# Nyrox/raymond

Measured on AMD Instinct MI355X. Metric: Msamples/s (whole node) + achieved HBM GB/s, 1920x1080 @ 500spp 5-bounce, higher is better.
Workload: dtype f64

## Files before the change

include/raymond_hip_probe.h:

```cpp
#ifndef RAYMOND_HIP_PROBE_H
#define RAYMOND_HIP_PROBE_H

#include "raymond_hip.h"

#ifdef __cplusplus
extern "C" {
#endif

rmd_status rmd_probe_philox4x32_10(rmd_context *ctx, size_t n, const uint32_t *ctr4, const uint32_t *key2, uint32_t *out4);
rmd_status rmd_probe_block_uniforms(rmd_context *ctx, uint64_t seed, size_t n, const uint32_t *pixel, const uint32_t *sample,
                                    const uint32_t *block, double *out5);
rmd_status rmd_probe_sphere_intersect(rmd_context *ctx, size_t n, const double *sphere4, const double *ray6, int32_t *hit, double *t);
rmd_status rmd_probe_sphere_normal(rmd_context *ctx, size_t n, const double *sphere4, const double *ray6, const double *t, double *n3);
rmd_status rmd_probe_plane_intersect(rmd_context *ctx, size_t n, const double *plane6, const double *ray6, int32_t *hit, double *t);
rmd_status rmd_probe_aabb_intersect(rmd_context *ctx, size_t n, const double *aabb6, const double *ray6, int32_t *hit, double *t);
rmd_status rmd_probe_triangle_intersect(rmd_context *ctx, size_t n, const double *pos9, const double *ray6, int32_t *hit, double *t);
rmd_status rmd_probe_triangle_normal(rmd_context *ctx, size_t n, const double *pos9, const double *nrm9, const double *ray6,
                                     const double *t, double *n3);
rmd_status rmd_probe_onb(rmd_context *ctx, size_t n, const double *n3, double *t3, double *b3);
rmd_status rmd_probe_cosine_hemisphere(rmd_context *ctx, size_t n, const double *r1, const double *r2, double *dir3, double *pdf);
rmd_status rmd_probe_importance_sample_ggx(rmd_context *ctx, size_t n, const double *reflect3, const double *rough, const double *r1,
                                           const double *r2, double *dir3);
rmd_status rmd_probe_ggx_distribution(rmd_context *ctx, size_t n, const double *n3, const double *h3, const double *rough, double *out);
rmd_status rmd_probe_geometry_smith(rmd_context *ctx, size_t n, const double *n3, const double *v3, const double *l3,
// ... 5 lines not shown
rmd_status rmd_probe_scene_intersect(rmd_context *ctx, const rmd_scene *scene, size_t n, const double *ray6, int32_t *obj, double *t,
                                     uint32_t *sub);
rmd_status rmd_probe_grid_intersect(rmd_context *ctx, const rmd_scene *scene, uint32_t g, size_t n, const double *ray6, int32_t *hit,
                                    double *t, uint32_t *tri);
rmd_status rmd_probe_grid_intersect_deep(rmd_context *ctx, const rmd_scene *scene, uint32_t g, size_t n, const double *ray6, uint32_t cut_lanes,
                                         uint32_t cut_round, uint32_t rays_per_wave, int32_t *hit, double *t, uint32_t *tri);
rmd_status rmd_probe_trace_samples(rmd_context *ctx, const rmd_scene *scene, const rmd_camera *cam, const rmd_settings *settings,
                                   size_t n, const uint32_t *xy2, const uint32_t *sample, double *rgb_out, int32_t *path_obj,
                                   uint32_t *path_sub);

rmd_status rmd_probe_triangle_sphere(size_t n, const double *pos9, double *out5);
rmd_status rmd_probe_primary_candidates(const rmd_camera *cam, const rmd_settings *settings, const rmd_object *objects, uint32_t n_objects, uint32_t n_grids,
                                        int64_t axis_pairs_tunable, size_t n_tiles, const uint32_t *tiles4, uint64_t *launch3, uint64_t *out2);
rmd_status rmd_probe_launch_plan(uint32_t mode, uint32_t grid, size_t n, const uint32_t *in5, uint64_t *out8);
rmd_status rmd_probe_launch_sizes(uint32_t mode, uint32_t grid, uint64_t *out8);
rmd_status rmd_probe_scene_layout(const rmd_scene *scene, uint32_t *n_objects, uint32_t *n_grids, uint32_t *mask_words_total);
#define RMD_PROBE_SCRATCH_FORMS 7u
#define RMD_PROBE_SCRATCH_PARTS 14u
rmd_status rmd_probe_denoise_scratch(uint32_t form, uint32_t width, uint32_t height, uint32_t n_rects, uint32_t guided, uint32_t n_cands, uint64_t n_table,
                                     uint64_t *out3, uint64_t *total);
rmd_status rmd_probe_pretest_pairs(rmd_context *ctx, size_t n, const double *sphere5, const double *pos9, const double *ray6, int32_t *pass,
                                   int32_t *hit, double *t);

#ifdef __cplusplus
}
#endif
#endif
```

raymond_amd/csrc/api.cpp:

```cpp
#define RMD_WITH_HIP 1
#include <algorithm>
#include <cmath>
#include <limits>
#include <cstdio>
#include <cstdlib>
#include <cstring>
#include <new>

#include "internal.hpp"
#include "launch.hpp"

using rmd::bind;

namespace {
thread_local std::string tl_last_error;

rmd_status context_create(int32_t device, hipStream_t stream, bool own_stream, rmd_context **out) {
	if (!out) return rmd::fail(nullptr, RMD_ERR_INVALID_ARGUMENT, "rmd_context_create: null out pointer");
	*out = nullptr;
	int count = 0;
	hipError_t e = hipGetDeviceCount(&count);
	if (e != hipSuccess || count <= 0)
		return rmd::fail(nullptr, RMD_ERR_NO_DEVICE, std::string("no HIP device: ") + (e != hipSuccess ? hipGetErrorString(e) : "device count is 0"));
	if (device < 0 || device >= count) return rmd::fail(nullptr, RMD_ERR_INVALID_ARGUMENT, "rmd_context_create: device ordinal out of range");
// ... 21 lines not shown
			return v ? (int64_t)std::atoll(v) : 0;
		};
		ctx->tunable[RMD_TUNE_SAMPLE_SPLIT] = env_int("RMD_SAMPLE_SPLIT");
		ctx->tunable[RMD_TUNE_WALK_BATCH] = env_int("RMD_WALK_BATCH");
		ctx->tunable[RMD_TUNE_MASK_BUDGET] = env_int("RMD_MASK_BUDGET");
		ctx->tunable[RMD_TUNE_SCRATCH_CAP_MB] = env_int("RMD_SCRATCH_CAP_MB");
		ctx->tunable[RMD_TUNE_WALK_CUT] = env_int("RMD_WALK_CUT");
		ctx->tunable[RMD_TUNE_SPLIT_MIN_SAMPLES] = env_int("RMD_SPLIT_MIN_SAMPLES");
		ctx->tunable[RMD_TUNE_CHAIN_ITEMS] = env_int("RMD_CHAIN_ITEMS");
		ctx->tunable[RMD_TUNE_AXIS_PAIRS] = env_int("RMD_AXIS_PAIRS");
		ctx->tunable[RMD_TUNE_PATH_QUEUES] = env_int("RMD_PATH_QUEUES");
		const char *form = std::getenv("RMD_LAUNCH_FORM");
		ctx->tunable[RMD_TUNE_LAUNCH_FORM] = !form ? 0 : (std::strcmp(form, "per-item") == 0 || std::strcmp(form, "1") == 0) ? 1 : (std::strcmp(form, "persistent") == 0 || std::strcmp(form, "2") == 0) ? 2 : 0;
#if RMD_DIAG
		ctx->debug_flags = (uint32_t)env_int("RMD_DEBUG");
#endif
	}
	if (hipEventCreate(&ctx->ev_start) != hipSuccess || hipEventCreate(&ctx->ev_stop) != hipSuccess)
		return rmd::fail(nullptr, RMD_ERR_HIP, "hipEventCreate failed");
	{
		void *h = nullptr, *d = nullptr;
		hipError_t fe = hipHostMalloc(&h, rmd::kFaultWords * sizeof(uint32_t), hipHostMallocMapped);
		if (fe == hipSuccess) {
			ctx->h_fault = (uint32_t *)h;
			std::memset(h, 0, rmd::kFaultWords * sizeof(uint32_t));
			fe = hipHostGetDevicePointer(&d, h, 0);
		}
		if (fe != hipSuccess) return rmd::fail(nullptr, RMD_ERR_HIP, std::string("fault words (hipHostMalloc): ") + hipGetErrorString(fe));
		ctx->d_fault = (uint32_t *)d;
	}
// ... 532 lines not shown
		const uint32_t waves_per_slot = has_grid ? 256u : 24u;
		k = (waves_per_slot * ctx->wave_slots + n_wave_tiles - 1u) / n_wave_tiles;
		if (has_grid && k < 2u) k = 2u;
		uint32_t min_samples = has_grid ? (sample_count <= rmd::kChainMaxSamples && ctx->tunable[RMD_TUNE_CHAIN_ITEMS] != 1 ? 2u : rmd::kSplitMinSamplesGrid) : 64u;
		if (ctx->tunable[RMD_TUNE_SPLIT_MIN_SAMPLES] > 0) min_samples = (uint32_t)std::min<int64_t>(ctx->tunable[RMD_TUNE_SPLIT_MIN_SAMPLES], 1 << 20);
		if (k > sample_count / min_samples) k = sample_count / min_samples;
		if (has_grid && k < 2u && sample_count >= 4u && ctx->tunable[RMD_TUNE_SPLIT_MIN_SAMPLES] <= 0) k = 2u;
	}
	if (k > 64u) k = 64u;
	while (k > 1u && (uint64_t)n_wave_tiles * k > 0x7FFFFFFFull) k--;
	if (k < 2u) k = 1u;
	if (buffered) *buffered = k > 1u || may_buffer_unsplit;
	return k;
}

static rmd_status render_tiles_async_impl(rmd_context *ctx, const rmd_scene *scene, const rmd_camera *camera, const rmd_settings *settings,
                                          const rmd_tile_rect *tiles, uint32_t n_tiles, double *accum_dev, double *accum_sq_dev) {
	if (rmd_status s = bind(ctx)) return s;
	if (rmd_status s = check_render_args(ctx, scene, camera, settings)) return s;
	if (!accum_dev || (n_tiles && !tiles)) return rmd::fail(ctx, RMD_ERR_INVALID_ARGUMENT, "rmd_render_tiles: null tiles/accum pointer");
	if (rmd_status s = prepare_wave_tiles(ctx, camera, tiles, n_tiles)) return s;
	if (settings->bounce_limit == 0u) {
		RMD_HIP(ctx, hipEventRecord(ctx->ev_start, ctx->stream));
		RMD_HIP(ctx, hipEventRecord(ctx->ev_stop, ctx->stream));
		ctx->timed = true;
		return RMD_OK;
	}
	rmd::RenderParams P = rmd::make_params(ctx, scene, camera, settings);
	P.n_work = ctx->n_wave_tiles;
	if (P.debug_flags & 24u) {
// ... 32 lines not shown
			if (e != hipErrorOutOfMemory) return rmd::fail(ctx, RMD_ERR_HIP, std::string("hipMalloc(sample scratch): ") + hipGetErrorString(e));
			if (per_pass <= 8u) {
				split = 1u, buffered = false, per_pass = P.sample_count;
				break;
			}
			per_pass = per_pass / 2u < 8u ? 8u : per_pass / 2u;
		}
	}
	ctx->last_launch = rmd_launch_info{};
	ctx->last_launch.end_black_paths = P.end_black_paths, ctx->last_launch.has_grid = scene->n_grids != 0u;
	RMD_HIP(ctx, hipEventRecord(ctx->ev_start, ctx->stream));
	for (uint64_t done = 0; done < settings->sample_count || done == 0; done += per_pass) {
		rmd::RenderParams Q = P;
		Q.sample_begin = settings->sample_begin + (uint32_t)done;
		Q.sample_count = settings->sample_count - done < per_pass ? (uint32_t)(settings->sample_count - done) : per_pass;
		Q.split_k = split > 1u ? choose_split(ctx, scene->n_grids != 0, P.n_work, Q.sample_count) : 1u;
		Q.sample_magic = Q.sample_count > 1u ? ~0ull / Q.sample_count + 1ull : 0ull;
		Q.buffered = buffered ? 1u : 0u;
		{
			const int64_t force = ctx->tunable[RMD_TUNE_CHAIN_ITEMS];
			Q.chain_items = (buffered && scene->n_grids != 0u && (force == 2 || (force == 0 && Q.sample_count <= rmd::kChainMaxSamples))) ? 1u : 0u;
		}
		Q.sample_buf = ctx->sample_buf.as<double>();
		const bool persistent_pass = persistent && ((uint64_t)P.n_work * Q.split_k >= ctx->wave_slots || ctx->tunable[RMD_TUNE_LAUNCH_FORM] == 2);
		if (persistent_pass) {
			RMD_HIP(ctx, hipMemsetAsync(ctx->work_counter.as<void>(), 0, sizeof(uint32_t), ctx->stream));
			Q.work_counter = ctx->work_counter.as<uint32_t>();
		}
		if (persistent_pass && buffered && scene->n_grids != 0u && ctx->tunable[RMD_TUNE_PATH_QUEUES] != 1) {
			const size_t wave_bytes = rmd::path_queue_bytes_host(rmd::kQueuePaths), need = wave_bytes * ctx->wave_slots;
			if (ctx->queue_buf.bytes() < need) {
				const hipError_t qe = (ctx->debug_flags & 256u) ? hipErrorOutOfMemory : ctx->queue_buf.grow(need);
				if (qe == hipSuccess) {
					RMD_HIP(ctx, hipMemsetAsync(ctx->queue_buf.as<void>(), 0, need, ctx->stream));
				} else {
					(void)hipGetLastError();
					if (qe != hipErrorOutOfMemory) return rmd::fail(ctx, RMD_ERR_HIP, std::string("hipMalloc(path queues): ") + hipGetErrorString(qe));
				}
			}
// ... 370 lines not shown
```

raymond_amd/csrc/device_types.hpp:

```cpp
#pragma once
#include <stdint.h>

namespace rmd {

struct alignas(16) DevObject {
	uint32_t geometry_kind;
	uint32_t grid_index;
	uint32_t material_kind;
	uint32_t pair_info;
	double origin[3];
	double radius;
	double normal[3];
	double roughness;
	double color[3];
	double metalness;
	uint32_t flags;
	uint32_t _pad2;
	double partner_origin_k;
};
constexpr uint32_t kObjBlackDiffuse = 1u;
constexpr uint32_t kObjAxisPair = 2u, kObjAxisShift = 8u, kObjAxisEarlierIsPlus = 1u << 10;
static_assert(sizeof(DevObject) == 128, "DevObject layout");
constexpr uint32_t kPairTestedAtPartner = 0x80000000u;
constexpr uint32_t kPairAxis = 0x40000000u;
// ... 60 lines not shown
	uint32_t walk_batch;
	uint32_t mask_words_total;
	uint32_t split_k;
	double *sample_buf;
	uint32_t debug_flags;
	unsigned long long *debug_counters;
	uint32_t *work_counter;
	uint32_t *tile_done;
	uint32_t end_black_paths;
	uint32_t walk_cut;
	uint32_t shade_last_depth;
	uint32_t chain_items;
	uint32_t primary_cull;
	uint32_t buffered;
	uint32_t axis_pairs;
	uint32_t _pad2;
	uint32_t *fault;
	unsigned char *queue_buf;
	uint32_t queue_wave_bytes;
	uint32_t queue_paths;
	uint32_t walk_steps_bound;
	uint32_t _pad3;
	unsigned long long visit_mask;
	unsigned long long grid_mask;
	unsigned long long sample_magic;
};
constexpr uint32_t kFaultTripLoop = 1u;
constexpr uint32_t kFaultSortedTripLoop = 2u;
constexpr uint32_t kFaultWorkLoop = 4u;
constexpr uint32_t kFaultWalkRounds = 8u;
constexpr uint32_t kFaultQueuedTripLoop = 16u;
// ... 9 lines not shown
```

raymond_amd/csrc/internal.hpp:

```cpp
#pragma once
#include <stdint.h>

#include <cmath>
#include <limits>
#include <algorithm>
#include <cstring>

#include <memory>
#include <mutex>
#include <string>
#include <vector>

#include "../../include/raymond_hip.h"

#ifdef RMD_WITH_HIP
#include <hip/hip_runtime_api.h>

#include "device_types.hpp"
#include "primary_candidates.hpp"

#define RMD_HIP(ctx, call)                                                                                      \
	do {                                                                                                        \
		hipError_t e_ = (call);                                                                                 \
		if (e_ != hipSuccess) return rmd::fail(ctx, e_ == hipErrorOutOfMemory ? RMD_ERR_OUT_OF_MEMORY : RMD_ERR_HIP, \
		                                       std::string(#call) + ": " + hipGetErrorString(e_));              \
	} while (0)

namespace rmd {
class DeviceBuffer {
public:
	DeviceBuffer() = default;
	DeviceBuffer(DeviceBuffer &&o) noexcept : p_(o.p_), bytes_(o.bytes_) { o.p_ = nullptr, o.bytes_ = 0; }
	DeviceBuffer &operator=(DeviceBuffer &&o) noexcept {
		if (this != &o) (void)release(), p_ = o.p_, bytes_ = o.bytes_, o.p_ = nullptr, o.bytes_ = 0;
// ... 42 lines not shown
	rmd::DeviceBuffer tile_done;
	rmd::DeviceBuffer debug_counters;
	rmd::DeviceBuffer atrous_region_scratch;
	uint32_t *h_fault = nullptr, *d_fault = nullptr;
	struct TransferSlot {
		rmd::DeviceBuffer packed;
		rmd::DeviceBuffer table;
		hipEvent_t packed_ready = nullptr, copied = nullptr;
		bool in_flight = false;
		std::vector<unsigned char> h_table;
	} transfer[2];
	uint32_t next_transfer = 0;
	hipStream_t copy_stream = nullptr;
	int64_t tunable[RMD_TUNE_COUNT] = {};
	uint32_t debug_flags = 0;
	rmd_launch_info last_launch = {};
	~rmd_context();
};

struct rmd_scene {
	rmd_context *ctx = nullptr;
	uint32_t n_objects = 0, n_grids = 0;
	uint32_t n_grid_objects = 0;
	uint32_t mask_words_total = 0;
	uint32_t axis_pairs = 0;
	unsigned long long visit_mask = ~0ull, grid_mask = ~0ull;
	uint32_t walk_steps_bound = 0;
	bool primary_cull = false;
	bool regular = true;
	rmd::DevObject *d_objects = nullptr;
// ... 82 lines not shown
		return body();
	} catch (const std::bad_alloc &) {
		return fail_noexcept(ctx, RMD_ERR_OUT_OF_MEMORY, what, "the host ran out of memory");
	} catch (const std::exception &e) {
		return fail_noexcept(ctx, RMD_ERR_HIP, what, e.what());
	} catch (...) {
		return fail_noexcept(ctx, RMD_ERR_HIP, what, "unknown exception");
	}
}
#ifdef RMD_WITH_HIP
rmd_status bind(rmd_context *ctx);
bool denoise_rects_ok(const rmd_tile_rect *rects, uint32_t n_rects, uint32_t width, uint32_t height, const char **why);
rmd_status check_fault(rmd_context *ctx);
RenderParams make_params(const rmd_context *ctx, const rmd_scene *scene, const rmd_camera *cam, const rmd_settings *st);
bool primary_cull_allowed(const RenderParams &P);
struct SceneObjects {
	std::vector<DevObject> objs;
	bool regular = true;
	uint32_t axis_pairs = 0;
	AxisWalls walls[3] = {};
	unsigned long long visit_mask = 0ull, grid_mask = 0ull;
};
rmd_status derive_scene_objects(rmd_context *ctx, const rmd_object *objects, uint32_t n_objects, uint32_t n_grids, int64_t axis_pairs_tunable, SceneObjects &out);
#endif
}
```

raymond_amd/csrc/kernels.hip:

```cpp
#include <hip/hip_runtime.h>

#include "render_kernel.hpp"

namespace rmd {

__global__ __launch_bounds__(64) void sum_kernel(RenderParams P, const WaveTile *__restrict__ tiles, const double *__restrict__ buf,
                                                 double *__restrict__ out) {
	const uint32_t wt = blockIdx.x, lane = threadIdx.x;
	const WaveTile t = tiles[wt];
	const uint32_t lx = lane & 7u, ly = lane >> 3;
	if (lx >= t.w || ly >= t.h) return;
	const size_t pix = ((size_t)(t.x0 + lx) + (size_t)(t.y0 + ly) * P.W) * 3;
	V3 acc = ld3(out + pix);
	const double *src = buf + ((size_t)wt * P.sample_count * 64u + lane) * kSampleStride;
	for (uint32_t s = 0; s < P.sample_count; s++) {
		acc = acc + ld3(src);
		src += 64u * kSampleStride;
	}
	out[pix + 0] = acc.x, out[pix + 1] = acc.y, out[pix + 2] = acc.z;
}

__global__ __launch_bounds__(64) void sum_moments_kernel(RenderParams P, const WaveTile *__restrict__ tiles, const double *__restrict__ buf,
                                                         double *__restrict__ out, double *__restrict__ out_sq) {
	const uint32_t wt = blockIdx.x, lane = threadIdx.x;
// ... 120 lines not shown
	switch (mode * 2 + (grid ? 1 : 0)) {
	case kModeTiles * 2: return lds_sizes_of<kModeTiles, false>(out);
	case kModeTiles * 2 + 1: return lds_sizes_of<kModeTiles, true>(out);
	case kModeTilesBuffered * 2: return lds_sizes_of<kModeTilesBuffered, false>(out);
	case kModeTilesBuffered * 2 + 1: return lds_sizes_of<kModeTilesBuffered, true>(out);
	case kModeList * 2: return lds_sizes_of<kModeList, false>(out);
	case kModeList * 2 + 1: return lds_sizes_of<kModeList, true>(out);
	}
	for (int i = 0; i < 8; i++) out[i] = 0;
}

hipError_t launch_render_tiles(hipStream_t stream, const RenderParams &P, const DevObject *objs, const DevGrid *grids,
                               const WaveTile *wave_tiles, double *accum, uint32_t n_cus, LaunchShape *shape, double *accum_sq) {
	if (P.n_work == 0) return hipSuccess;
	const bool buffered = P.buffered != 0u;
	const uint32_t n_waves = P.n_work * (buffered ? P.split_k : 1u);
	hipError_t e;
	if (P.n_grids) e = buffered ? launch_render<kModeTilesBuffered, true>(stream, P, objs, grids, wave_tiles, n_waves, accum, nullptr, nullptr, n_cus, shape)
	                            : launch_render<kModeTiles, true>(stream, P, objs, grids, wave_tiles, n_waves, accum, nullptr, nullptr, n_cus, shape, accum_sq);
	else e = buffered ? launch_render<kModeTilesBuffered, false>(stream, P, objs, grids, wave_tiles, n_waves, accum, nullptr, nullptr, n_cus, shape, accum_sq)
	                  : launch_render<kModeTiles, false>(stream, P, objs, grids, wave_tiles, n_waves, accum, nullptr, nullptr, n_cus, shape, accum_sq);
	if (e != hipSuccess || !buffered || P.tile_done != nullptr) return e;
	if (accum_sq) hipLaunchKernelGGL(sum_moments_kernel, dim3(P.n_work), dim3(64), 0, stream, P, wave_tiles, (const double *)P.sample_buf, accum, accum_sq);
	else hipLaunchKernelGGL(sum_kernel, dim3(P.n_work), dim3(64), 0, stream, P, wave_tiles, (const double *)P.sample_buf, accum);
	return hipGetLastError();
}

hipError_t launch_sum(hipStream_t stream, const RenderParams &P, const WaveTile *wave_tiles, double *accum) {
	if (P.n_work == 0) return hipSuccess;
	hipLaunchKernelGGL(sum_kernel, dim3(P.n_work), dim3(64), 0, stream, P, wave_tiles, (const double *)P.sample_buf, accum);
	return hipGetLastError();
// ... 12 lines not shown
```

raymond_amd/csrc/probe.cpp:

```cpp
#define RMD_WITH_HIP 1
#include <cstring>
#include <vector>

#include "../../include/raymond_hip_probe.h"
#include "internal.hpp"
#include "launch.hpp"

namespace {

struct Column {
	const double *src;
	int width;
};

rmd_status run_probe(rmd_context *ctx, int op, size_t n, const std::vector<Column> &cols, int out_stride, std::vector<double> &out,
                     const rmd::RenderParams *params = nullptr) {
	if (!ctx) return rmd::fail(nullptr, RMD_ERR_INVALID_ARGUMENT, "probe: null context");
	RMD_HIP(ctx, hipSetDevice(ctx->device));
	int in_stride = 0;
	for (const Column &c : cols) {
		if (!c.src && n) return rmd::fail(ctx, RMD_ERR_INVALID_ARGUMENT, "probe: null input array");
		in_stride += c.width;
	}
	std::vector<double> in(n * in_stride);
// ... 243 lines not shown
	});
}

rmd_status rmd_probe_launch_plan(uint32_t mode, uint32_t grid, size_t n, const uint32_t *in5, uint64_t *out8) {
	if (mode > 2u || grid > 1u || (n != 0 && (!in5 || !out8))) return rmd::fail(nullptr, RMD_ERR_INVALID_ARGUMENT, "probe: bad argument");
	for (size_t i = 0; i < n; i++) {
		const uint32_t *a = in5 + i * 5;
		const rmd::LaunchPlan L = rmd::plan_render_launch((int)mode, grid != 0u, a[0], a[1], (a[2] & 1u) != 0u, (a[2] & 2u) != 0u, (a[2] & 4u) != 0u,
		                                                  (a[2] & 8u) != 0u, a[3], a[4]);
		uint64_t *o = out8 + i * 8;
		o[0] = L.persistent, o[1] = L.queued, o[2] = L.chained, o[3] = L.moments, o[4] = L.waves_per_wg, o[5] = L.workgroups, o[6] = L.wave_lds, o[7] = L.lds;
	}
	return RMD_OK;
}

rmd_status rmd_probe_launch_sizes(uint32_t mode, uint32_t grid, uint64_t *out8) {
	if (mode > 2u || grid > 1u || !out8) return rmd::fail(nullptr, RMD_ERR_INVALID_ARGUMENT, "probe: bad argument");
	rmd::render_lds_sizes((int)mode, grid != 0u, out8);
	return RMD_OK;
}

static_assert(RMD_PROBE_SCRATCH_FORMS == rmd::kScratchForms && RMD_PROBE_SCRATCH_PARTS == rmd::kScratchParts, "include/raymond_hip_probe.h mirrors denoise_host.hpp");
rmd_status rmd_probe_denoise_scratch(uint32_t form, uint32_t width, uint32_t height, uint32_t n_rects, uint32_t guided, uint32_t n_cands, uint64_t n_table,
                                     uint64_t *out3, uint64_t *total) {
	if (form >= rmd::kScratchForms || guided > 1u || !out3 || !total) return rmd::fail(nullptr, RMD_ERR_INVALID_ARGUMENT, "probe: bad argument");
	const rmd::ScratchLayout L = rmd::denoise_scratch_layout((rmd::ScratchForm)form, width, height, n_rects, guided != 0u, n_cands, (size_t)n_table);
	for (uint32_t p = 0; p < rmd::kScratchParts; p++) out3[3 * p] = L.used[p], out3[3 * p + 1] = L.offset[p], out3[3 * p + 2] = L.bytes[p];
	*total = L.total;
	return RMD_OK;
}
// ... 54 lines not shown
```

raymond_amd/csrc/render_kernel.hpp:

```cpp
#pragma once
#include <hip/hip_runtime.h>

#include "device_core.hpp"
#include "grid_walk.hpp"
#include "launch.hpp"
#include "lobe_trips.hpp"
#include "primary_candidates.hpp"
#include "scene_split.hpp"

namespace rmd {

struct alignas(16) PathId {
	uint32_t px[64];
	uint32_t smp[64];
	uint32_t sector[64];
};
__host__ __device__ inline size_t wave_lds_bytes(uint32_t n_grids) { return kWaveHeadBytes + (n_grids ? sizeof(WalkScratch) + 64u * 3u * sizeof(double) + sizeof(WalkCarry) + sizeof(PathId) : 0); }

RMD_DEV uint32_t work_item_of_block(uint32_t b, uint32_t nb) {
	(void)nb;
	return b;
}

RMD_DEV void report_fault(const RenderParams &P, uint32_t code, uint32_t detail) {
// ... 74 lines not shown
	}
	t_best = closest;
	sub_best = sub;
	return best;
}

constexpr uint32_t kWalkMinRunnable = 24;
constexpr uint32_t kWalkMaxWait = 6;
constexpr uint32_t kWalkCutMinWalkers = 16;
constexpr uint32_t kWalkCutMinRunnable = 0;

constexpr uint32_t kGridMinWaves = 4, kNoGridMinWaves = 3;
enum { kModeTiles = 0, kModeTilesBuffered = 1, kModeList = 2 };
RMD_DEV void store_sample(RMD_GLOBAL double *dst, V3 L) { dst[0] = L.x, dst[1] = L.y, dst[2] = L.z; }
template <bool MOM = false>
RMD_DEV void finish_sample_range(const RenderParams &P, const WaveTile &tile, uint32_t wt, uint32_t lane, double *__restrict__ out, double *__restrict__ out_sq = nullptr) {
	if (P.tile_done == nullptr || wt >= P.n_work) return;
	__builtin_amdgcn_fence(__ATOMIC_RELEASE, "agent");
	uint32_t before = 0;
	if (lane == 0u) before = __hip_atomic_fetch_add(P.tile_done + wt, 1u, __ATOMIC_RELAXED, __HIP_MEMORY_SCOPE_AGENT);
	before = (uint32_t)__builtin_amdgcn_readfirstlane((int)before);
	if (before + 1u != P.split_k) return;
	__builtin_amdgcn_fence(__ATOMIC_ACQUIRE, "agent");
	const uint32_t lx = lane & 7u, ly = lane >> 3;
	if (lx < tile.w && ly < tile.h) {
		const size_t pix = ((size_t)(tile.x0 + lx) + (size_t)(tile.y0 + ly) * P.W) * 3;
		V3 sum = ld3(out + pix);
		[[maybe_unused]] V3 sq = mk(0.0, 0.0, 0.0);
		if constexpr (MOM) sq = ld3(out_sq + pix);
		const RMD_GLOBAL double *src = (const RMD_GLOBAL double *)P.sample_buf + ((size_t)wt * P.sample_count * 64u + lane) * kSampleStride;
		constexpr uint32_t kInFlight = MOM ? 8u : 16u;
		uint32_t k = 0;
		for (; k + kInFlight <= P.sample_count; k += kInFlight) {
			V3 v[kInFlight];
#pragma unroll
			for (uint32_t j = 0; j < kInFlight; j++) v[j] = ld3(src + (size_t)j * 64u * kSampleStride);
#pragma unroll
			for (uint32_t j = 0; j < kInFlight; j++) {
// ... 362 lines not shown
			complete = want && !waiting;
			t = part_t, oi = part_obj, sub = part_sub;
		} else {
			oi = scene_intersect_wave<false>(objs, Pt.n_objects, grids, lds_masks, scr, want, ro, rd, t, sub, Pt.axis_pairs, Pt.debug_flags, Pt.debug_counters, false, Pt.visit_mask);
			complete = want;
		}
	}

#if RMD_DIAG
	if (tstamp && lane == 0) {
		atomicAdd(&P.debug_counters[0], __builtin_amdgcn_s_memtime() - tt_begin), atomicAdd(&P.debug_counters[1], tt_b);
		atomicAdd(&P.debug_counters[2], tt_simple), atomicAdd(&P.debug_counters[3], tt_walk), atomicAdd(&P.debug_counters[4], tt_class);
	}
#endif
#undef RMD_TSTAMP
	if constexpr (to_buffer && !GRID) finish_sample_range(P, tile, wt, lane, out);
	if (writes && !to_buffer && !acc_in_memory) {
		out[out_index + 0] = acc.x;
		out[out_index + 1] = acc.y;
		out[out_index + 2] = acc.z;
		if constexpr (MOM && !acc_in_memory) out_sq[out_index + 0] = acc_sq.x, out_sq[out_index + 1] = acc_sq.y, out_sq[out_index + 2] = acc_sq.z;
	}
}

constexpr int kSortObjPrio = 1;
struct alignas(16) HitStack {
	double frag[3][kSortSlots], T[3][kSortSlots];
	uint32_t state[kSortSlots];
	uint32_t lobe_bits[kSortSlots];
	uint32_t item[kSortSlots];
};
// ... 26 lines not shown
		pairs = primary_pairs_kept(cone, cc, w3, P.axis_pairs);
	}
	if (lane == 0u) sets[0] = pairs, sets[1] = (uint32_t)visit, sets[2] = (uint32_t)(visit >> 32);
	__builtin_amdgcn_fence(__ATOMIC_RELEASE, "wavefront");
	__builtin_amdgcn_wave_barrier();
	__builtin_amdgcn_fence(__ATOMIC_ACQUIRE, "wavefront");
}
#define RMD_UNDEF3(v) RMD_UNDEF(v.x) RMD_UNDEF(v.y) RMD_UNDEF(v.z)
template <bool MOM = false>
RMD_DEV void render_wave_sorted(const RenderParams &P, KernargWords kernarg_params, const DevObject *__restrict__ objs, const DevGrid *__restrict__ grids,
                                const void *__restrict__ work, double *__restrict__ out, const DevObject *lobjs, unsigned char *wave_lds, uint32_t work_item,
                                double *__restrict__ out_sq = nullptr) {
	const uint32_t lane = threadIdx.x & 63u;
	HitStack &stack = *reinterpret_cast<HitStack *>(wave_lds);
	WalkScratch *no_scratch = nullptr;
	const uint32_t wt = work_item / P.split_k, part = work_item % P.split_k;
	const bool have = wt < P.n_work;
	const WaveTile tile = reinterpret_cast<const WaveTile *>(work)[have ? wt : 0];
	const uint32_t per_part = (P.sample_count + P.split_k - 1u) / P.split_k;
	const uint32_t s_lo = part * per_part < P.sample_count ? part * per_part : P.sample_count;
	const uint32_t s_hi = s_lo + per_part < P.sample_count ? s_lo + per_part : P.sample_count;
	const uint32_t pool_first = s_lo, pool_items = have ? (s_hi - s_lo) * 64u : 0u;
	if (P.bounce_limit == 0u) return;
	const V3 cam_pos = ld3(P.cam_pos);

	uint32_t *item_sets = reinterpret_cast<uint32_t *>(wave_lds + sizeof(HitStack)) + 1;
	item_candidates(kernarg_params, tile, objs, lobjs, item_sets);

	uint32_t n_d = 0, n_g = 0, next_item = 0;
	unsigned long long trips_left = lobe_trip_bound(pool_items, kTripBoundPerPair);
#if RMD_DIAG
	if (P.debug_flags & 32u) trips_left = 1ull;
#endif
	for (;;) {
		KernargWords src = kernarg_params;
		asm volatile("" : "+s"(src));
		unsigned long long w[sizeof(RenderParams) / 8];
// ... 137 lines not shown
				stack.frag[0][e] = frag.x, stack.frag[1][e] = frag.y, stack.frag[2][e] = frag.z;
				stack.T[0][e] = T.x, stack.T[1][e] = T.y, stack.T[2][e] = T.z;
				stack.state[e] = (uint32_t)oi | (rng.block << 16);
				stack.lobe_bits[e] = rng.lobe_bits | (depth << 24), stack.item[e] = item;
			}
			n_d += (uint32_t)__popcll(pm_d), n_g += (uint32_t)__popcll(pm_g);
#if RMD_DIAG
			if ((Pt.debug_flags & 8u) && Pt.debug_counters && lane == 0u)
				atomicAdd(&Pt.debug_counters[41], (unsigned long long)__popcll(pm_d)), atomicAdd(&Pt.debug_counters[42], (unsigned long long)__popcll(pm_g));
#endif
			__builtin_amdgcn_fence(__ATOMIC_RELEASE, "wavefront");
			__builtin_amdgcn_wave_barrier();
			__builtin_amdgcn_fence(__ATOMIC_ACQUIRE, "wavefront");
		}
	}
	finish_sample_range<MOM>(P, tile, wt, lane, out, out_sq);
}

struct PathQueues {
	RMD_GLOBAL double *hit_d;
	RMD_GLOBAL double *ray_d;
	RMD_GLOBAL uint32_t *hit_w;
	RMD_GLOBAL uint32_t *ray_w;
	uint32_t cap;
};
constexpr uint32_t kRayCarried = 1u << 23;
__host__ __device__ inline size_t path_queue_bytes(uint32_t cap) { return (size_t)cap * (9u * 8u + 13u * 8u + 4u * 4u + 9u * 4u); }
RMD_DEV uint32_t sample_of_sector(const RenderParams &P, uint32_t sector) {
	const uint32_t a = sector >> 6, q = (uint32_t)__umul64hi((unsigned long long)a, P.sample_magic);
	return P.sample_begin + (P.sample_magic != 0ull ? a - q * P.sample_count : 0u);
}
// ... 390 lines not shown
	[[maybe_unused]] unsigned char *wave_head = wave_lds + wave_lds_of<MODE, GRID, QUEUED>(P.n_grids) - kWaveHeadBytes;
	{
		const double *src = reinterpret_cast<const double *>(objs);
		double *dst = reinterpret_cast<double *>(lobjs);
		for (uint32_t i = tid; i < P.n_objects * 16u; i += blockDim.x) dst[i] = src[i];
		for (uint32_t gi = 0; gi < P.n_grids; gi++) {
			const DevGrid &g = grids[gi];
			if (g.mask_lds_word == 0xFFFFFFFFu) continue;
			for (uint32_t i = tid; i < g.mask_n_words; i += blockDim.x) lmasks[g.mask_lds_word + i] = as_global(g.mask_words)[i];
		}
	}
	__syncthreads();
	const uint32_t *lds_masks = P.mask_words_total ? lmasks : nullptr;
	if constexpr (PERSIST) {
		static_assert(MODE != kModeList, "list launches are not persistent");
		const uint32_t n_items = P.n_work * (MODE == kModeTilesBuffered ? P.split_k : 1u);
		volatile uint32_t *last_draw = reinterpret_cast<volatile uint32_t *>(wave_head);
		if ((tid & 63u) == 0u) *last_draw = 0u;
		for (;;) {
			uint32_t item = 0, floor = 0;
			if ((tid & 63u) == 0u) {
				item = atomicAdd(P.work_counter, 1u);
				floor = *last_draw;
				*last_draw = item + 1u;
#if RMD_DIAG
				if ((P.debug_flags & 128u) && floor != 0u) floor = 0xFFFFFFFFu;
#endif
			}
			item = (uint32_t)__builtin_amdgcn_readfirstlane((int)item);
			if (item >= n_items) break;
			floor = (uint32_t)__builtin_amdgcn_readfirstlane((int)floor);
// ... 106 lines not shown
```

raymond_amd/probe.py:

```python
import ctypes as C
import os

import numpy as np

from . import abi
from . import lib as _lib

_vp = C.c_void_p
_sz = C.c_size_t
_P = C.POINTER
_SIGS = {
    "rmd_probe_philox4x32_10": [_vp, _sz, _vp, _vp, _vp],
    "rmd_probe_block_uniforms": [_vp, C.c_uint64, _sz, _vp, _vp, _vp, _vp],
    "rmd_probe_sphere_intersect": [_vp, _sz, _vp, _vp, _vp, _vp],
    "rmd_probe_sphere_normal": [_vp, _sz, _vp, _vp, _vp, _vp],
    "rmd_probe_plane_intersect": [_vp, _sz, _vp, _vp, _vp, _vp],
    "rmd_probe_aabb_intersect": [_vp, _sz, _vp, _vp, _vp, _vp],
    "rmd_probe_triangle_intersect": [_vp, _sz, _vp, _vp, _vp, _vp],
    "rmd_probe_triangle_normal": [_vp, _sz, _vp, _vp, _vp, _vp, _vp],
    "rmd_probe_onb": [_vp, _sz, _vp, _vp, _vp],
    "rmd_probe_cosine_hemisphere": [_vp, _sz, _vp, _vp, _vp, _vp],
    "rmd_probe_importance_sample_ggx": [_vp, _sz, _vp, _vp, _vp, _vp, _vp],
    "rmd_probe_ggx_distribution": [_vp, _sz, _vp, _vp, _vp, _vp],
    "rmd_probe_geometry_smith": [_vp, _sz, _vp, _vp, _vp, _vp, _vp],
    "rmd_probe_fresnel_schlick": [_vp, _sz, _vp, _vp, _vp],
    "rmd_probe_primary_ray": [_vp, _sz, _P(abi.Camera), _vp, _vp, _vp],
    "rmd_probe_elementary": [_vp, _sz, _vp, _vp, _vp, _vp, _vp, _vp],
    "rmd_probe_scene_intersect": [_vp, _vp, _sz, _vp, _vp, _vp, _vp],
    "rmd_probe_grid_intersect": [_vp, _vp, C.c_uint32, _sz, _vp, _vp, _vp, _vp],
    "rmd_probe_grid_intersect_deep": [_vp, _vp, C.c_uint32, _sz, _vp, C.c_uint32, C.c_uint32, C.c_uint32, _vp, _vp, _vp],
    "rmd_probe_trace_samples": [_vp, _vp, _P(abi.Camera), _P(abi.Settings), _sz, _vp, _vp, _vp, _vp, _vp],
    "rmd_probe_triangle_sphere": [_sz, _vp, _vp],
    "rmd_probe_pretest_pairs": [_vp, _sz, _vp, _vp, _vp, _vp, _vp, _vp],
    "rmd_probe_primary_candidates": [_P(abi.Camera), _P(abi.Settings), _P(abi.Object), C.c_uint32, C.c_uint32, C.c_int64, _sz, _vp, _vp, _vp],
    "rmd_probe_launch_plan": [C.c_uint32, C.c_uint32, _sz, _vp, _vp],
    "rmd_probe_launch_sizes": [C.c_uint32, C.c_uint32, _vp],
    "rmd_probe_scene_layout": [_vp, _P(C.c_uint32), _P(C.c_uint32), _P(C.c_uint32)],
    "rmd_probe_denoise_scratch": [C.c_uint32] * 6 + [C.c_uint64, _vp, _P(C.c_uint64)],
}
PATH_STRIDE = 17
_ready = False


PROBE_LIB_PATH = os.path.join(os.path.dirname(_lib.LIB_PATH), "libraymond_hip_probe.so")
_probe_lib = None


def _L():
    global _ready, _probe_lib
    if not _ready:
        _lib.load()
# ... 168 lines not shown
    L = _L()
    cols = np.broadcast_arrays(*(np.asarray(a, dtype=np.int64) for a in (n_objects, mask_words_total, flags, n_waves, n_cus)))
    inp = np.ascontiguousarray(np.stack([c.ravel() for c in cols], axis=1).astype(np.uint32))
    out = np.zeros((inp.shape[0], 8), dtype=np.uint64)
    _host_check(L.rmd_probe_launch_plan(mode, int(grid), inp.shape[0], _p(inp), _p(out)), "rmd_probe_launch_plan")
    return {k: out[:, i].astype(np.int64).reshape(cols[0].shape) for i, k in enumerate(PLAN_FIELDS)}


def launch_sizes(mode, grid):
    L = _L()
    out = np.zeros(8, dtype=np.uint64)
    _host_check(L.rmd_probe_launch_sizes(mode, int(grid), _p(out)), "rmd_probe_launch_sizes")
    return {k: int(v) for k, v in zip(SIZE_FIELDS, out)}


def scene_layout(dscene):
    L = _L()
    n, g, m = C.c_uint32(), C.c_uint32(), C.c_uint32()
    _host_check(L.rmd_probe_scene_layout(dscene.handle, C.byref(n), C.byref(g), C.byref(m)), "rmd_probe_scene_layout")
    return n.value, g.value, m.value


SCRATCH_FORMS = ("single", "atrous", "dual", "atrous_dual", "atrous_dual_region", "dual_select", "tile_error")
SCRATCH_PARTS = ("planes", "f_b", "cand_img", "gain", "feat_planes", "n_img", "win_img", "n_f_img", "table", "rects", "counts_a", "counts_b", "counts_f",
                 "tile_errors")


def denoise_scratch(form, width, height, n_rects, guided=False, n_cands=0, n_table=0):
    L = _L()
    out = np.zeros((len(SCRATCH_PARTS), 3), dtype=np.uint64)
# ... 5 lines not shown
```

Measured before the change: 25360.

## Split only tail tiles across sample parts in persistent buffered launches

Adds a work-list plan where most tiles run as whole items (all samples, one wave) and only a tail set of tiles, sized relative to wave slots, is split into k sample parts. Whole items skip the agent-scope atomic completion counter and use only wavefront-scope fences. The aim is to cut split overhead and atomics while keeping load balance at the end of a persistent launch. It applies only to buffered, non-grid, persistent passes, which adds planning complexity and possible tail imbalance.

Result: faster. 26310, median of 6 (+3.7%).

```diff
diff --git a/include/raymond_hip_probe.h b/include/raymond_hip_probe.h
--- a/include/raymond_hip_probe.h
+++ b/include/raymond_hip_probe.h
@@ -43,6 +43,9 @@
                                         int64_t axis_pairs_tunable, size_t n_tiles, const uint32_t *tiles4, uint64_t *launch3, uint64_t *out2);
 rmd_status rmd_probe_launch_plan(uint32_t mode, uint32_t grid, size_t n, const uint32_t *in5, uint64_t *out8);
 rmd_status rmd_probe_launch_sizes(uint32_t mode, uint32_t grid, uint64_t *out8);
+rmd_status rmd_probe_work_plan(const rmd_context *ctx, size_t n, const uint32_t *in4, uint32_t *out3);
+rmd_status rmd_probe_work_items(uint32_t n_tiles, uint32_t n_whole, uint32_t k_tail, uint32_t sample_count, uint32_t first, size_t n, uint32_t *out5,
+                                uint32_t *n_items);
 rmd_status rmd_probe_scene_layout(const rmd_scene *scene, uint32_t *n_objects, uint32_t *n_grids, uint32_t *mask_words_total);
 #define RMD_PROBE_SCRATCH_FORMS 7u
 #define RMD_PROBE_SCRATCH_PARTS 14u
diff --git a/raymond_amd/csrc/api.cpp b/raymond_amd/csrc/api.cpp
--- a/raymond_amd/csrc/api.cpp
+++ b/raymond_amd/csrc/api.cpp
@@ -59,6 +59,12 @@
 		ctx->tunable[RMD_TUNE_LAUNCH_FORM] = !form ? 0 : (std::strcmp(form, "per-item") == 0 || std::strcmp(form, "1") == 0) ? 1 : (std::strcmp(form, "persistent") == 0 || std::strcmp(form, "2") == 0) ? 2 : 0;
 #if RMD_DIAG
 		ctx->debug_flags = (uint32_t)env_int("RMD_DEBUG");
+#endif
+#if RMD_WORK_LIST_SWEEP
+		if (const char *v = std::getenv("RMD_WORK_LIST")) {
+			unsigned a = 0, b = 0;
+			if (std::sscanf(v, "%u,%u", &a, &b) == 2 && b >= 1u) ctx->tail_x2 = a, ctx->tail_parts = b;
+		}
 #endif
 	}
 	if (hipEventCreate(&ctx->ev_start) != hipSuccess || hipEventCreate(&ctx->ev_stop) != hipSuccess)
@@ -621,6 +627,42 @@
 	return k;
 }
 
+extern "C++" {
+namespace rmd {
+WorkPlan plan_work_list(uint32_t wave_slots, uint32_t n_tiles, uint32_t sample_count, uint32_t k_uniform, uint32_t min_samples, uint32_t tail_x2, uint32_t tail_parts,
+                        uint32_t n_tail_forced) {
+	WorkPlan w{0u, n_tiles, k_uniform < 1u ? 1u : k_uniform};
+	if (tail_x2 == 0u || sample_count > kWholeMaxSamples) return w;
+	const uint64_t n_tail = n_tail_forced ? (uint64_t)n_tail_forced : ((uint64_t)tail_x2 * wave_slots + 1u) / 2u;
+	if ((uint64_t)n_tiles <= n_tail) return w;
+	uint32_t k = tail_parts > 64u ? 64u : tail_parts;
+	if (min_samples < 1u) min_samples = 1u;
+	if (k > sample_count / min_samples) k = sample_count / min_samples;
+	if (k < w.k_tail) k = w.k_tail;
+	if ((uint64_t)(n_tiles - n_tail) + n_tail * k > 0x7FFFFFFFull) return w;
+	w.n_whole = n_tiles - (uint32_t)n_tail, w.n_tail = (uint32_t)n_tail, w.k_tail = k;
+	return w;
+}
+static WorkPlan pass_work_plan(const rmd_context *ctx, bool has_grid, bool split_launch, bool buffered, bool persistent, uint32_t n_tiles, uint32_t sample_count,
+                               bool *persistent_pass) {
+	WorkPlan w{0u, n_tiles, split_launch ? choose_split(ctx, has_grid, n_tiles, sample_count) : 1u};
+	*persistent_pass = persistent && ((uint64_t)n_tiles * w.k_tail >= ctx->wave_slots || ctx->tunable[RMD_TUNE_LAUNCH_FORM] == 2);
+	if (!buffered || has_grid || !*persistent_pass || ctx->tunable[RMD_TUNE_SAMPLE_SPLIT] > 0) return w;
+	uint32_t min_samples = kTailMinSamples, forced_tail = 0u;
+	if (ctx->tunable[RMD_TUNE_SPLIT_MIN_SAMPLES] > 0) min_samples = (uint32_t)std::min<int64_t>(ctx->tunable[RMD_TUNE_SPLIT_MIN_SAMPLES], 1 << 20);
+#if RMD_DIAG
+	if (ctx->debug_flags & 1024u) forced_tail = 4u;
+#endif
+	return plan_work_list(ctx->wave_slots, n_tiles, sample_count, w.k_tail, min_samples, ctx->tail_x2, ctx->tail_parts, forced_tail);
+}
+WorkPlan context_work_plan(const rmd_context *ctx, bool has_grid, uint32_t n_tiles, uint32_t sample_count, uint32_t pass_samples) {
+	bool buffered = false, persistent_pass = false;
+	const uint32_t split = choose_split(ctx, has_grid, n_tiles, sample_count, &buffered);
+	return pass_work_plan(ctx, has_grid, split > 1u, buffered, ctx->tunable[RMD_TUNE_LAUNCH_FORM] != 1, n_tiles, pass_samples, &persistent_pass);
+}
+}
+}
+
 static rmd_status render_tiles_async_impl(rmd_context *ctx, const rmd_scene *scene, const rmd_camera *camera, const rmd_settings *settings,
                                           const rmd_tile_rect *tiles, uint32_t n_tiles, double *accum_dev, double *accum_sq_dev) {
 	if (rmd_status s = bind(ctx)) return s;
@@ -683,7 +725,9 @@
 		rmd::RenderParams Q = P;
 		Q.sample_begin = settings->sample_begin + (uint32_t)done;
 		Q.sample_count = settings->sample_count - done < per_pass ? (uint32_t)(settings->sample_count - done) : per_pass;
-		Q.split_k = split > 1u ? choose_split(ctx, scene->n_grids != 0, P.n_work, Q.sample_count) : 1u;
+		bool persistent_pass = false;
+		const rmd::WorkPlan list = rmd::pass_work_plan(ctx, scene->n_grids != 0, split > 1u, buffered, persistent, P.n_work, Q.sample_count, &persistent_pass);
+		Q.split_k = list.k_tail, Q.n_whole = list.n_whole;
 		Q.sample_magic = Q.sample_count > 1u ? ~0ull / Q.sample_count + 1ull : 0ull;
 		Q.buffered = buffered ? 1u : 0u;
 		{
@@ -691,7 +735,6 @@
 			Q.chain_items = (buffered && scene->n_grids != 0u && (force == 2 || (force == 0 && Q.sample_count <= rmd::kChainMaxSamples))) ? 1u : 0u;
 		}
 		Q.sample_buf = ctx->sample_buf.as<double>();
-		const bool persistent_pass = persistent && ((uint64_t)P.n_work * Q.split_k >= ctx->wave_slots || ctx->tunable[RMD_TUNE_LAUNCH_FORM] == 2);
 		if (persistent_pass) {
 			RMD_HIP(ctx, hipMemsetAsync(ctx->work_counter.as<void>(), 0, sizeof(uint32_t), ctx->stream));
 			Q.work_counter = ctx->work_counter.as<uint32_t>();
diff --git a/raymond_amd/csrc/device_types.hpp b/raymond_amd/csrc/device_types.hpp
--- a/raymond_amd/csrc/device_types.hpp
+++ b/raymond_amd/csrc/device_types.hpp
@@ -98,7 +98,7 @@
 	uint32_t primary_cull;
 	uint32_t buffered;
 	uint32_t axis_pairs;
-	uint32_t _pad2;
+	uint32_t n_whole;
 	uint32_t *fault;
 	unsigned char *queue_buf;
 	uint32_t queue_wave_bytes;
diff --git a/raymond_amd/csrc/internal.hpp b/raymond_amd/csrc/internal.hpp
--- a/raymond_amd/csrc/internal.hpp
+++ b/raymond_amd/csrc/internal.hpp
@@ -18,6 +18,7 @@
 
 #include "device_types.hpp"
 #include "primary_candidates.hpp"
+#include "work_list.hpp"
 
 #define RMD_HIP(ctx, call)                                                                                      \
 	do {                                                                                                        \
@@ -90,6 +91,7 @@
 	hipStream_t copy_stream = nullptr;
 	int64_t tunable[RMD_TUNE_COUNT] = {};
 	uint32_t debug_flags = 0;
+	uint32_t tail_x2 = rmd::kTailTilesPerSlotX2, tail_parts = rmd::kTailParts;
 	rmd_launch_info last_launch = {};
 	~rmd_context();
 };
@@ -202,6 +204,9 @@
 rmd_status check_fault(rmd_context *ctx);
 RenderParams make_params(const rmd_context *ctx, const rmd_scene *scene, const rmd_camera *cam, const rmd_settings *st);
 bool primary_cull_allowed(const RenderParams &P);
+WorkPlan plan_work_list(uint32_t wave_slots, uint32_t n_tiles, uint32_t sample_count, uint32_t k_uniform, uint32_t min_samples = kTailMinSamples,
+                        uint32_t tail_x2 = kTailTilesPerSlotX2, uint32_t tail_parts = kTailParts, uint32_t n_tail_forced = 0u);
+WorkPlan context_work_plan(const rmd_context *ctx, bool has_grid, uint32_t n_tiles, uint32_t sample_count, uint32_t pass_samples);
 struct SceneObjects {
 	std::vector<DevObject> objs;
 	bool regular = true;
diff --git a/raymond_amd/csrc/kernels.hip b/raymond_amd/csrc/kernels.hip
--- a/raymond_amd/csrc/kernels.hip
+++ b/raymond_amd/csrc/kernels.hip
@@ -158,7 +158,7 @@
                                const WaveTile *wave_tiles, double *accum, uint32_t n_cus, LaunchShape *shape, double *accum_sq) {
 	if (P.n_work == 0) return hipSuccess;
 	const bool buffered = P.buffered != 0u;
-	const uint32_t n_waves = P.n_work * (buffered ? P.split_k : 1u);
+	const uint32_t n_waves = buffered ? work_list_items(P.n_work, P.n_whole, P.split_k) : P.n_work;
 	hipError_t e;
 	if (P.n_grids) e = buffered ? launch_render<kModeTilesBuffered, true>(stream, P, objs, grids, wave_tiles, n_waves, accum, nullptr, nullptr, n_cus, shape)
 	                            : launch_render<kModeTiles, true>(stream, P, objs, grids, wave_tiles, n_waves, accum, nullptr, nullptr, n_cus, shape, accum_sq);
diff --git a/raymond_amd/csrc/probe.cpp b/raymond_amd/csrc/probe.cpp
--- a/raymond_amd/csrc/probe.cpp
+++ b/raymond_amd/csrc/probe.cpp
@@ -281,6 +281,28 @@
 	return RMD_OK;
 }
 
+rmd_status rmd_probe_work_plan(const rmd_context *ctx, size_t n, const uint32_t *in4, uint32_t *out3) {
+	if (n != 0 && (!in4 || !out3)) return rmd::fail(nullptr, RMD_ERR_INVALID_ARGUMENT, "probe: bad argument");
+	for (size_t i = 0; i < n; i++) {
+		const uint32_t *a = in4 + i * 4;
+		const rmd::WorkPlan w = ctx ? rmd::context_work_plan(ctx, false, a[1], a[2], a[0] ? a[0] : a[2]) : rmd::plan_work_list(a[0], a[1], a[2], a[3]);
+		out3[i * 3] = w.n_whole, out3[i * 3 + 1] = w.n_tail, out3[i * 3 + 2] = w.k_tail;
+	}
+	return RMD_OK;
+}
+
+rmd_status rmd_probe_work_items(uint32_t n_tiles, uint32_t n_whole, uint32_t k_tail, uint32_t sample_count, uint32_t first, size_t n, uint32_t *out5,
+                                uint32_t *n_items) {
+	if (n_whole > n_tiles || k_tail == 0u || !n_items || (n != 0 && !out5)) return rmd::fail(nullptr, RMD_ERR_INVALID_ARGUMENT, "probe: bad argument");
+	*n_items = rmd::work_list_items(n_tiles, n_whole, k_tail);
+	for (size_t i = 0; i < n; i++) {
+		const rmd::WorkItem w = rmd::work_list_item(first + (uint32_t)i, n_tiles, n_whole, k_tail, sample_count);
+		uint32_t *o = out5 + i * 5;
+		o[0] = w.tile, o[1] = w.first, o[2] = w.count, o[3] = w.parts, o[4] = w.whole;
+	}
+	return RMD_OK;
+}
+
 rmd_status rmd_probe_launch_sizes(uint32_t mode, uint32_t grid, uint64_t *out8) {
 	if (mode > 2u || grid > 1u || !out8) return rmd::fail(nullptr, RMD_ERR_INVALID_ARGUMENT, "probe: bad argument");
 	rmd::render_lds_sizes((int)mode, grid != 0u, out8);
diff --git a/raymond_amd/csrc/render_kernel.hpp b/raymond_amd/csrc/render_kernel.hpp
--- a/raymond_amd/csrc/render_kernel.hpp
+++ b/raymond_amd/csrc/render_kernel.hpp
@@ -7,6 +7,7 @@
 #include "lobe_trips.hpp"
 #include "primary_candidates.hpp"
 #include "scene_split.hpp"
+#include "work_list.hpp"
 
 namespace rmd {
 
@@ -112,14 +113,22 @@
 enum { kModeTiles = 0, kModeTilesBuffered = 1, kModeList = 2 };
 RMD_DEV void store_sample(RMD_GLOBAL double *dst, V3 L) { dst[0] = L.x, dst[1] = L.y, dst[2] = L.z; }
 template <bool MOM = false>
-RMD_DEV void finish_sample_range(const RenderParams &P, const WaveTile &tile, uint32_t wt, uint32_t lane, double *__restrict__ out, double *__restrict__ out_sq = nullptr) {
+RMD_DEV void finish_sample_range(const RenderParams &P, const WaveTile &tile, uint32_t wt, uint32_t parts, bool whole, uint32_t lane, double *__restrict__ out,
+                                 double *__restrict__ out_sq = nullptr) {
 	if (P.tile_done == nullptr || wt >= P.n_work) return;
-	__builtin_amdgcn_fence(__ATOMIC_RELEASE, "agent");
-	uint32_t before = 0;
-	if (lane == 0u) before = __hip_atomic_fetch_add(P.tile_done + wt, 1u, __ATOMIC_RELAXED, __HIP_MEMORY_SCOPE_AGENT);
-	before = (uint32_t)__builtin_amdgcn_readfirstlane((int)before);
-	if (before + 1u != P.split_k) return;
-	__builtin_amdgcn_fence(__ATOMIC_ACQUIRE, "agent");
+	if (whole) {
+		__builtin_amdgcn_fence(__ATOMIC_RELEASE, "wavefront");
+		__builtin_amdgcn_s_waitcnt(0);
+		__builtin_amdgcn_wave_barrier();
+		__builtin_amdgcn_fence(__ATOMIC_ACQUIRE, "wavefront");
+	} else {
+		__builtin_amdgcn_fence(__ATOMIC_RELEASE, "agent");
+		uint32_t before = 0;
+		if (lane == 0u) before = __hip_atomic_fetch_add(P.tile_done + wt, 1u, __ATOMIC_RELAXED, __HIP_MEMORY_SCOPE_AGENT);
+		before = (uint32_t)__builtin_amdgcn_readfirstlane((int)before);
+		if (before + 1u != parts) return;
+		__builtin_amdgcn_fence(__ATOMIC_ACQUIRE, "agent");
+	}
 	const uint32_t lx = lane & 7u, ly = lane >> 3;
 	if (lx < tile.w && ly < tile.h) {
 		const size_t pix = ((size_t)(tile.x0 + lx) + (size_t)(tile.y0 + ly) * P.W) * 3;
@@ -512,7 +521,7 @@
 	}
 #endif
 #undef RMD_TSTAMP
-	if constexpr (to_buffer && !GRID) finish_sample_range(P, tile, wt, lane, out);
+	if constexpr (to_buffer && !GRID) finish_sample_range(P, tile, wt, P.split_k, false, lane, out);
 	if (writes && !to_buffer && !acc_in_memory) {
 		out[out_index + 0] = acc.x;
 		out[out_index + 1] = acc.y;
@@ -569,13 +578,11 @@
 	const uint32_t lane = threadIdx.x & 63u;
 	HitStack &stack = *reinterpret_cast<HitStack *>(wave_lds);
 	WalkScratch *no_scratch = nullptr;
-	const uint32_t wt = work_item / P.split_k, part = work_item % P.split_k;
+	const WorkItem wi = work_list_item(work_item, P.n_work, P.n_whole, P.split_k, P.sample_count);
+	const uint32_t wt = wi.tile;
 	const bool have = wt < P.n_work;
 	const WaveTile tile = reinterpret_cast<const WaveTile *>(work)[have ? wt : 0];
-	const uint32_t per_part = (P.sample_count + P.split_k - 1u) / P.split_k;
-	const uint32_t s_lo = part * per_part < P.sample_count ? part * per_part : P.sample_count;
-	const uint32_t s_hi = s_lo + per_part < P.sample_count ? s_lo + per_part : P.sample_count;
-	const uint32_t pool_first = s_lo, pool_items = have ? (s_hi - s_lo) * 64u : 0u;
+	const uint32_t pool_first = wi.first, pool_items = wi.count * 64u;
 	if (P.bounce_limit == 0u) return;
 	const V3 cam_pos = ld3(P.cam_pos);
 
@@ -743,7 +750,7 @@
 			__builtin_amdgcn_fence(__ATOMIC_ACQUIRE, "wavefront");
 		}
 	}
-	finish_sample_range<MOM>(P, tile, wt, lane, out, out_sq);
+	finish_sample_range<MOM>(P, tile, wt, P.split_k, work_item < P.n_whole, lane, out, out_sq);
 }
 
 struct PathQueues {
@@ -1164,7 +1171,7 @@
 	const uint32_t *lds_masks = P.mask_words_total ? lmasks : nullptr;
 	if constexpr (PERSIST) {
 		static_assert(MODE != kModeList, "list launches are not persistent");
-		const uint32_t n_items = P.n_work * (MODE == kModeTilesBuffered ? P.split_k : 1u);
+		const uint32_t n_items = kSortedTrips<MODE, GRID> ? work_list_items(P.n_work, P.n_whole, P.split_k) : P.n_work * (MODE == kModeTilesBuffered ? P.split_k : 1u);
 		volatile uint32_t *last_draw = reinterpret_cast<volatile uint32_t *>(wave_head);
 		if ((tid & 63u) == 0u) *last_draw = 0u;
 		for (;;) {
diff --git a/raymond_amd/csrc/work_list.hpp b/raymond_amd/csrc/work_list.hpp
--- /dev/null
+++ b/raymond_amd/csrc/work_list.hpp
@@ -0,0 +1,43 @@
+#pragma once
+#include <stdint.h>
+
+#if defined(__HIP__)
+#define RMD_WORK_HD __host__ __device__ inline
+#else
+#define RMD_WORK_HD inline
+#endif
+
+namespace rmd {
+
+struct WorkItem {
+	uint32_t tile;
+	uint32_t first;
+	uint32_t count;
+	uint32_t parts;
+	uint32_t whole;
+};
+RMD_WORK_HD uint32_t work_list_items(uint32_t n_tiles, uint32_t n_whole, uint32_t k_tail) { return n_whole + (n_tiles - n_whole) * k_tail; }
+RMD_WORK_HD WorkItem work_list_item(uint32_t item, uint32_t n_tiles, uint32_t n_whole, uint32_t k_tail, uint32_t sample_count) {
+	WorkItem w;
+	if (item < n_whole) {
+		w.tile = item, w.first = 0u, w.count = sample_count, w.parts = 1u, w.whole = 1u;
+	} else {
+		const uint32_t t = item - n_whole, q = t / k_tail, part = t - q * k_tail;
+		const uint32_t per_part = (sample_count + k_tail - 1u) / k_tail;
+		const uint32_t s_lo = part * per_part < sample_count ? part * per_part : sample_count;
+		const uint32_t s_hi = s_lo + per_part < sample_count ? s_lo + per_part : sample_count;
+		w.tile = n_whole + q, w.first = s_lo, w.count = s_hi - s_lo, w.parts = k_tail, w.whole = 0u;
+	}
+	if (w.tile >= n_tiles) w.tile = n_tiles, w.count = 0u;
+	return w;
+}
+
+struct WorkPlan {
+	uint32_t n_whole, n_tail, k_tail;
+};
+constexpr uint32_t kWholeMaxSamples = 1u << 20;
+constexpr uint32_t kTailTilesPerSlotX2 = 5u;
+constexpr uint32_t kTailParts = 4u;
+constexpr uint32_t kTailMinSamples = 64u;
+
+}
diff --git a/raymond_amd/probe.py b/raymond_amd/probe.py
--- a/raymond_amd/probe.py
+++ b/raymond_amd/probe.py
@@ -35,6 +35,8 @@
     "rmd_probe_primary_candidates": [_P(abi.Camera), _P(abi.Settings), _P(abi.Object), C.c_uint32, C.c_uint32, C.c_int64, _sz, _vp, _vp, _vp],
     "rmd_probe_launch_plan": [C.c_uint32, C.c_uint32, _sz, _vp, _vp],
     "rmd_probe_launch_sizes": [C.c_uint32, C.c_uint32, _vp],
+    "rmd_probe_work_plan": [_vp, _sz, _vp, _vp],
+    "rmd_probe_work_items": [C.c_uint32, C.c_uint32, C.c_uint32, C.c_uint32, C.c_uint32, _sz, _vp, _P(C.c_uint32)],
     "rmd_probe_scene_layout": [_vp, _P(C.c_uint32), _P(C.c_uint32), _P(C.c_uint32)],
     "rmd_probe_denoise_scratch": [C.c_uint32] * 6 + [C.c_uint64, _vp, _P(C.c_uint64)],
 }
@@ -233,6 +235,29 @@
     return {k: int(v) for k, v in zip(SIZE_FIELDS, out)}
 
 
+def work_plan(wave_slots, n_tiles, sample_count, k_uniform, ctx=None, pass_samples=0):
+    L = _L()
+    if ctx is not None:
+        wave_slots = pass_samples
+    cols = np.broadcast_arrays(*(np.asarray(a, dtype=np.int64) for a in (wave_slots, n_tiles, sample_count, k_uniform)))
+    inp = np.ascontiguousarray(np.stack([c.ravel() for c in cols], axis=1).astype(np.uint32))
+    out = np.zeros((inp.shape[0], 3), dtype=np.uint32)
+    _host_check(L.rmd_probe_work_plan(ctx.handle if ctx is not None else None, inp.shape[0], _p(inp), _p(out)), "rmd_probe_work_plan")
+    return tuple(out[:, i].astype(np.int64).reshape(cols[0].shape) for i in range(3))
+
+
+WORK_ITEM_FIELDS = ("tile", "first", "count", "parts", "whole")
+
+
+def work_items(n_tiles, n_whole, k_tail, sample_count, extra=0):
+    L = _L()
+    n_items = C.c_uint32()
+    _host_check(L.rmd_probe_work_items(n_tiles, n_whole, k_tail, sample_count, 0, 0, None, C.byref(n_items)), "rmd_probe_work_items")
+    out = np.zeros((n_items.value + extra, 5), dtype=np.uint32)
+    _host_check(L.rmd_probe_work_items(n_tiles, n_whole, k_tail, sample_count, 0, out.shape[0], _p(out), C.byref(n_items)), "rmd_probe_work_items")
+    return out.astype(np.int64), n_items.value
+
+
 def scene_layout(dscene):
     L = _L()
     n, g, m = C.c_uint32(), C.c_uint32(), C.c_uint32()
```
